# feixue94/pram

Hardware: AMD Instinct MI355X
Metric: query images/sec (640x480, 2048 kpts, 7Scenes nc113) (higher is better)
Workload: dtype f32 results via split-fp16 MFMA (f16 x3 products, f32 accumulate); 1 GPU; 7Scenes full hot path: SFD2 extract+sample -> SegNetViT nc113 (15 layers) -> GML match + 20 Sinkhorn iters, 2048 query kpts vs a 2048-kpt reference set; stages=erm; precision=x3, batches_in_flight_per_gpu=3, hipgraph_replay=False, attention_chunk_keys=4096, frame=640x480, keypoints=2048, parallelism=query-sharded x1, one all-gather of result records, matches_last_step=14291, matches_correct_last_step=14288, gather_order_verified=True

## Files before the change

### pram_amd/csrc/gemm_core_x3w.h

```cpp
#pragma once
#include "common.h"
#include "gemm_core_x3.h"
#include <type_traits>

namespace gemmx3w {

using gemmx3::half4;
using gemmx3::half8;
using gemmx3::split4;
using gemmx3::swz;

constexpr int BK = 32;
#ifndef PRAM_GEMM_SHADOW
#define PRAM_GEMM_SHADOW 1
#endif
constexpr bool SHADOW = PRAM_GEMM_SHADOW != 0;

static __device__ unsigned long long prof[72];

template <int MI, int WM, int WN>
struct Cfg {
    static constexpr int NT = 64 * WM * WN;
    static constexpr int BM = WM * 32 * MI;
    static constexpr int BN = WN * 64;
    static constexpr int PA = BM * 8 / NT;
    static constexpr int QA = BM * 4 / NT;
    static constexpr int QB = BN * 4 / NT;
    static constexpr int RA = NT / 8;
    static constexpr int RQ = NT / 4;
};

template <int MI, int WM, int WN>
struct alignas(16) Smem {
    using C = Cfg<MI, WM, WN>;
    _Float16 ah[2][C::BM * BK];
    _Float16 al[2][C::BM * BK];
    _Float16 bh[2][C::BN * BK];
    _Float16 bl[2][C::BN * BK];
};

template <int ROWS, int NWAVES, class RowPtr>
__device__ __forceinline__ void dma_tile(_Float16* lds_hi, _Float16* lds_lo, RowPtr& rowptr) {
    const int lane = threadIdx.x & 63, wave = threadIdx.x >> 6;
    constexpr int PIECES = ROWS / 16;
#pragma unroll
    for (int i = 0; i < (2 * PIECES + NWAVES - 1) / NWAVES; ++i) {
        const int piece = wave + NWAVES * i;
        if (piece < 2 * PIECES) {
            const int plane = piece / PIECES, pc = piece % PIECES;
            const int row = pc * 16 + (lane >> 2);
            const int slot = (lane & 3) ^ ((row >> 2) & 3);
            const _Float16* src = rowptr(row, plane) + slot * 8;
            _Float16* dst = (plane ? lds_lo : lds_hi) + pc * 16 * BK;
            __builtin_amdgcn_global_load_lds(src, dst, 16, 0, 0);
        }
    }
}

template <int MI, int WM, int WN, bool APLANES, int ABL, int DMA, class Adv, class ALoad, class AOk, class BLoad, class BOk, class APtr, class BPtr, class AXf>
__device__ __forceinline__ void mainloop(Smem<MI, WM, WN>& s, Adv& adv, ALoad& la, AOk& oka, BLoad& lb, BOk& okb, APtr& aptr, BPtr& bptr,
                                         int nk, float a_scale, f32x16 (&acc)[MI][2], float& amax, AXf& axf);

template <int MI, int WM, int WN, bool APLANES, int ABL, int DMA, class Adv, class ALoad, class AOk, class BLoad, class BOk, class APtr, class BPtr>
__device__ __forceinline__ void mainloop(Smem<MI, WM, WN>& s, Adv& adv, ALoad& la, AOk& oka, BLoad& lb, BOk& okb, APtr& aptr, BPtr& bptr,
                                         int nk, float a_scale, f32x16 (&acc)[MI][2], float& amax) {
    gemmx3::NoXform none;
    mainloop<MI, WM, WN, APLANES, ABL, DMA>(s, adv, la, oka, lb, okb, aptr, bptr, nk, a_scale, acc, amax, none);
}

template <int MI, int WM, int WN, bool APLANES, int ABL, int DMA, class Adv, class ALoad, class AOk, class BLoad, class BOk, class APtr, class BPtr, class AXf>
__device__ __forceinline__ void mainloop(Smem<MI, WM, WN>& s, Adv& adv, ALoad& la, AOk& oka, BLoad& lb, BOk& okb, APtr& aptr, BPtr& bptr,
                                         int nk, float a_scale, f32x16 (&acc)[MI][2], float& amax, AXf& axf) {
    static_assert(DMA < 2 || APLANES, "A can only travel by DMA when it is already split");
    using C = Cfg<MI, WM, WN>;
    const int tid = threadIdx.x;
    const int lane = tid & 63, wave = tid >> 6;
    const int wm = wave / WN, wn = wave % WN;
    const int r = lane & 31, h = lane >> 5;
    const int arow = tid >> 3, akq = tid & 7;
    const int qrow = tid >> 2, qsl = tid & 3;

#pragma unroll
    for (int mi = 0; mi < MI; ++mi)
#pragma unroll
        for (int ni = 0; ni < 2; ++ni)
#pragma unroll
            for (int e = 0; e < 16; ++e) acc[mi][ni][e] = 0.f;

    constexpr int NA = APLANES ? C::QA : C::PA;
    struct Regs {
        float4 a[APLANES ? 1 : C::PA];
        uint4 ah[APLANES ? C::QA : 1], al[APLANES ? C::QA : 1];
        uint4 bh[C::QB], bl[C::QB];
        unsigned ok;
        int kt;
    };
    auto issue = [&](int kt, Regs& g) {
        g.ok = 0u;
        g.kt = kt;
        if constexpr (DMA < 2 && !(ABL & 16)) {
#pragma unroll
            for (int p = 0; p < NA; ++p) {
                if constexpr (APLANES) { g.ah[p] = la(p, kt, 0); g.al[p] = la(p, kt, 1); }
                else g.a[p] = la(p, kt);
                g.ok |= (oka(p, kt) ? 1u : 0u) << p;
            }
        }
        if constexpr (DMA < 1) {
#pragma unroll
            for (int p = 0; p < C::QB; ++p) { g.bh[p] = lb(p, kt, 0); g.bl[p] = lb(p, kt, 1); g.ok |= (okb(p, kt) ? 1u : 0u) << (8 + p); }
        }
    };
    auto dma = [&](int buf, int kt) {
        if constexpr (DMA >= 1 && !(ABL & 32)) {
            auto bp = [&](int row, int plane) { return bptr(row, plane, kt); };
            dma_tile<C::BN, C::NT / 64>(s.bh[buf], s.bl[buf], bp);
        }
        if constexpr (DMA >= 2) {
            auto ap = [&](int row, int plane) { return aptr(row, plane, kt); };
            dma_tile<C::BM, C::NT / 64>(s.ah[buf], s.al[buf], ap);
        }
    };
    auto dma_wait = [&]() {
        if constexpr (DMA >= 1) asm volatile("s_waitcnt vmcnt(0)" ::: "memory");
    };
    auto commit = [&](int buf, const Regs& g) {
#pragma unroll
        for (int p = 0; p < ((DMA < 2 && !(ABL & 16)) ? NA : 0); ++p) {
            if constexpr (APLANES) {
                const int row = qrow + C::RQ * p;
                uint4 vh = g.ah[p], vl = g.al[p];
                if (!((g.ok >> p) & 1u)) { vh = make_uint4(0u, 0u, 0u, 0u); vl = vh; }
                const int off = row * BK + swz(qsl, row) * 8;
                *reinterpret_cast<uint4*>(&s.ah[buf][off]) = vh;
                *reinterpret_cast<uint4*>(&s.al[buf][off]) = vl;
            } else {
                const int row = arow + C::RA * p;
                float4 v = g.a[p];
                if (!((g.ok >> p) & 1u)) v = make_float4(0.f, 0.f, 0.f, 0.f);
                else axf(v, p, g.kt);
                half4 hi, lo;
                split4(v, a_scale, hi, lo, amax);
                const int off = row * BK + swz(akq >> 1, row) * 8 + (akq & 1) * 4;
                *reinterpret_cast<half4*>(&s.ah[buf][off]) = hi;
                *reinterpret_cast<half4*>(&s.al[buf][off]) = lo;
            }
        }
#pragma unroll
        for (int p = 0; p < (DMA < 1 ? C::QB : 0); ++p) {
            const int row = qrow + C::RQ * p;
            uint4 vh = g.bh[p], vl = g.bl[p];
            if (!((g.ok >> (8 + p)) & 1u)) { vh = make_uint4(0u, 0u, 0u, 0u); vl = vh; }
            const int off = row * BK + swz(qsl, row) * 8;
            *reinterpret_cast<uint4*>(&s.bh[buf][off]) = vh;
            *reinterpret_cast<uint4*>(&s.bl[buf][off]) = vl;
        }
    };
    auto kstep = [&](int cur, int ks) {
        const int arow0 = (wm * 32 * MI + r) * BK, brow0 = (wn * 64 + r) * BK;
        const int slot = swz(2 * ks + h, r) * 8;
        half8 bh[2], bl[2], ah[2], al[2];
#pragma unroll
        for (int ni = 0; ni < 2; ++ni) {
            bh[ni] = *reinterpret_cast<const half8*>(&s.bh[cur][brow0 + ni * 32 * BK + slot]);
            bl[ni] = *reinterpret_cast<const half8*>(&s.bl[cur][brow0 + ni * 32 * BK + slot]);
        }
        ah[0] = *reinterpret_cast<const half8*>(&s.ah[cur][arow0 + slot]);
        al[0] = *reinterpret_cast<const half8*>(&s.al[cur][arow0 + slot]);
#pragma unroll
        for (int mi = 0; mi < MI; ++mi) {
            if (mi + 1 < MI) {
                ah[(mi + 1) & 1] = *reinterpret_cast<const half8*>(&s.ah[cur][arow0 + (mi + 1) * 32 * BK + slot]);
                al[(mi + 1) & 1] = *reinterpret_cast<const half8*>(&s.al[cur][arow0 + (mi + 1) * 32 * BK + slot]);
            }
            __builtin_amdgcn_sched_barrier(0);
#pragma unroll
            for (int ni = 0; ni < 2; ++ni) acc[mi][ni] = __builtin_amdgcn_mfma_f32_32x32x16_f16(al[mi & 1], bh[ni], acc[mi][ni], 0, 0, 0);
#pragma unroll
            for (int ni = 0; ni < 2; ++ni) acc[mi][ni] = __builtin_amdgcn_mfma_f32_32x32x16_f16(ah[mi & 1], bl[ni], acc[mi][ni], 0, 0, 0);
#pragma unroll
            for (int ni = 0; ni < 2; ++ni) acc[mi][ni] = __builtin_amdgcn_mfma_f32_32x32x16_f16(ah[mi & 1], bh[ni], acc[mi][ni], 0, 0, 0);
        }
    };

    if constexpr (MI <= 2) {
        Regs g0, g1;
        adv(0);
        issue(0, g0);
        dma(0, 0);
        if (nk > 1) { adv(1); issue(1, g1); }
        commit(0, g0);
        dma_wait();
        __syncthreads();
        auto step = [&](int kt, Regs& fresh, Regs& next) {
            if (kt + 1 < nk && !(ABL & 1)) dma((kt + 1) & 1, kt + 1);
            if (kt + 2 < nk && !(ABL & 1)) { adv(kt + 2); issue(kt + 2, fresh); }
            __builtin_amdgcn_sched_barrier(0);
            kstep(kt & 1, 0);
            kstep(kt & 1, (ABL & 2) ? 0 : 1);
            __builtin_amdgcn_sched_barrier(0);
            if (kt + 1 < nk && !(ABL & 1)) commit((kt + 1) & 1, next);
            dma_wait();
            __syncthreads();
        };
        for (int kt = 0; kt < nk; kt += 2) {
            step(kt, g0, g1);
            if (kt + 1 < nk) step(kt + 1, g1, g0);
        }
    } else if constexpr ((ABL == 0 || ABL >= 64) && SHADOW && DMA >= 1) {
        static_assert(MI == 4, "one staging piece per 32-row block of the 256-row tile");
        static_assert(2 * (C::BN / 16) <= (C::NT / 64) * MI && 2 * (C::BM / 16) <= (C::NT / 64) * MI, "MI DMA rounds cover the tile");
        Regs g;
        adv(0);
        issue(0, g);
        dma(0, 0);
        commit(0, g);
        dma_wait();
        __syncthreads();
        auto issue_piece = [&](int kt, int p) {
            if (p == 0) { g.ok = 0u; g.kt = kt; }
            if constexpr (DMA < 2) {
                if (p < NA) {
                    if constexpr (APLANES) { g.ah[p] = la(p, kt, 0); g.al[p] = la(p, kt, 1); }
                    else g.a[p] = la(p, kt);
                    g.ok |= (oka(p, kt) ? 1u : 0u) << p;
                }
            }
        };
        auto dma_piece = [&](int buf, int kt, int i) {
            const int wv = threadIdx.x >> 6, ln = threadIdx.x & 63;
            constexpr int NWV = C::NT / 64;
            {
                constexpr int PIECES = C::BN / 16;
                const int piece = wv + NWV * i;
                if (piece < 2 * PIECES) {
                    const int plane = piece / PIECES, pc = piece % PIECES;
                    const int row = pc * 16 + (ln >> 2);
                    const int slot = (ln & 3) ^ ((row >> 2) & 3);
                    __builtin_amdgcn_global_load_lds(bptr(row, plane, kt) + slot * 8, (plane ? s.bl[buf] : s.bh[buf]) + pc * 16 * BK, 16, 0, 0);
                }
            }
            if constexpr (DMA >= 2) {
                constexpr int PIECES = C::BM / 16;
                const int piece = wv + NWV * i;
                if (piece < 2 * PIECES) {
                    const int plane = piece / PIECES, pc = piece % PIECES;
                    const int row = pc * 16 + (ln >> 2);
                    const int slot = (ln & 3) ^ ((row >> 2) & 3);
                    __builtin_amdgcn_global_load_lds(aptr(row, plane, kt) + slot * 8, (plane ? s.al[buf] : s.ah[buf]) + pc * 16 * BK, 16, 0, 0);
                }
            }
        };
        auto commit_piece = [&](int buf, int p) {
            if (p >= NA) return;
            if constexpr (DMA < 2) {
                if constexpr (APLANES) {
                    const int row = qrow + C::RQ * p;
                    uint4 vh = g.ah[p], vl = g.al[p];
                    if (!((g.ok >> p) & 1u)) { vh = make_uint4(0u, 0u, 0u, 0u); vl = vh; }
                    const int off = row * BK + swz(qsl, row) * 8;
                    *reinterpret_cast<uint4*>(&s.ah[buf][off]) = vh;
                    *reinterpret_cast<uint4*>(&s.al[buf][off]) = vl;
                } else {
                    const int row = arow + C::RA * p;
                    float4 v = g.a[p];
                    if (!((g.ok >> p) & 1u)) v = make_float4(0.f, 0.f, 0.f, 0.f);
                    else axf(v, p, g.kt);
                    half4 hi, lo;
// ... 117 lines not shown
```

### pram_amd/csrc/linear.hip

```cpp
#include "gemm_core.h"
#include "gemm_core_f16.h"
#include "gemm_core_x3.h"
#include "gemm_core_x3w.h"
#include "launch.h"

namespace {

struct LinArgs {
    const float* a0; int lda0; int k0;
    const float* a1; int lda1; int k1;
    const float* w;
    const float* bias;
    const float* residual; int ldr;
    float* out; int ldo;
    int m, n;
    float alpha;
    int flags;
    const float* rcos; const float* rsin; int rot_cols;
    long long sa, sw, so;
    int tiles_m, tiles_n;
    void* out16; int ldo16;
    void* out16_lo; float out16_scale;
    const int* lens; int t_pad;
    void* vt_hi; void* vt_lo; int vt_col0, vt_heads, vt_t, vt_tv;
    unsigned int* status;
    float* row_ssq;
    const float* ln_ssq; int ln_parts; const float* ln_gamma; const float* ln_beta; float ln_eps;
    float act_scale = gemmx3::ACT_SCALE;
};

__device__ __forceinline__ float gelu_erf(float t) {
    const float a = fminf(fabsf(t), 6.0f);
    float q = fmaf(-3.327738795633195e-06f, a, 1.992317265830934e-06f);
    q = fmaf(q, a, 0.0006240683724172413f);
    q = fmaf(q, a, -0.0077792988158762455f);
    q = fmaf(q, a, 0.053078699856996536f);
    q = fmaf(q, a, 0.4589627683162689f);
    q = fmaf(q, a, 1.1511503458023071f);
    q = fmaf(q, a, 0.9999977350234985f);
    const float sgm = __builtin_amdgcn_exp2f(-q);
    return t * (t >= 0.f ? 1.0f - sgm : sgm);
}

template <int PA>
struct LnGeluXf {
    const float* gb; int K; int kq;
    float rstd[PA];
    __device__ __forceinline__ void operator()(float4& v, int p, int kt) const {
#if defined(PRAM_LNA_ABLATE) && (PRAM_LNA_ABLATE == 1 || PRAM_LNA_ABLATE == 4)
        (void)p; (void)kt;
#elif defined(PRAM_LNA_ABLATE) && PRAM_LNA_ABLATE == 2
        const int k = kt * 32 + kq * 4;
        const float4 g = *reinterpret_cast<const float4*>(gb + k);
        const float4 b = *reinterpret_cast<const float4*>(gb + K + k);
        const float rs = rstd[p];
        v.x = v.x * rs * g.x + b.x; v.y = v.y * rs * g.y + b.y; v.z = v.z * rs * g.z + b.z; v.w = v.w * rs * g.w + b.w;
#elif defined(PRAM_LNA_ABLATE) && PRAM_LNA_ABLATE == 3
        const float rs = rstd[p];
        (void)kt;
        v.x = gelu_erf(v.x * rs); v.y = gelu_erf(v.y * rs); v.z = gelu_erf(v.z * rs); v.w = gelu_erf(v.w * rs);
#else
        const int k = kt * 32 + kq * 4;
        const float4 g = *reinterpret_cast<const float4*>(gb + k);
        const float4 b = *reinterpret_cast<const float4*>(gb + K + k);
        const float rs = rstd[p];
        v.x = gelu_erf(v.x * rs * g.x + b.x);
        v.y = gelu_erf(v.y * rs * g.y + b.y);
        v.z = gelu_erf(v.z * rs * g.z + b.z);
        v.w = gelu_erf(v.w * rs * g.w + b.w);
#endif
    }
};

__device__ __forceinline__ float ln_rstd(const LinArgs& p, int row, int K) {
    constexpr int QMAX = 16;
    float s = 0.f;
    for (int q0 = 0; q0 < p.ln_parts; q0 += QMAX) {
        float v[QMAX];
#pragma unroll
        for (int i = 0; i < QMAX; ++i) v[i] = p.ln_ssq[(size_t)min(q0 + i, p.ln_parts - 1) * p.m + row];
#pragma unroll
        for (int i = 0; i < QMAX; ++i)
            if (q0 + i < p.ln_parts) s += v[i];
    }
    return 1.0f / sqrtf(s / (float)K + p.ln_eps);
}

__device__ __forceinline__ bool tile_has_rows(const int* __restrict__ lens, int t_pad, int row0, int bm, int m) {
    if (!lens) return true;
    const int rend = min(row0 + bm, m);
    for (int s = row0 / t_pad; s * t_pad < rend; ++s)
        if (max(row0, s * t_pad) - s * t_pad < lens[s]) return true;
    return false;
}

__device__ __forceinline__ bool row_valid(const int* __restrict__ lens, int t_pad, int row, int m) {
    if (row >= m) return false;
    if (!lens) return true;
    const int sq = row / t_pad;
    return row - sq * t_pad < lens[sq];
}

template <int MI, int WN>
__device__ __forceinline__ void linear_epilogue(const LinArgs& p, f32x16 (&acc)[MI][2], float* out, int row0, int col0,
                                                int BM, int BN, _Float16* stage = nullptr) {
    using gemm::acc_row;
    const int tid = threadIdx.x;
    const int mlast = p.m - 1, nlast = p.n - 1;
    const int lane = tid & 63, wave = __builtin_amdgcn_readfirstlane(tid >> 6);
    const int wm = wave / WN, wn = wave % WN;
    const int r = lane & 31, h = lane >> 5;
    const int cbase = col0 + wn * 64;
    const bool rot = (p.flags & PRAM_LIN_ROTARY) && cbase < p.rot_cols;
    const int c0 = cbase + r, c1 = cbase + 32 + r;
    const bool c0ok = c0 < p.n, c1ok = c1 < p.n;
    const int c0c = min(c0, nlast), c1c = min(c1, nlast);
    const float b0 = p.bias ? p.bias[c0c] : 0.f, b1 = p.bias ? p.bias[c1c] : 0.f;
    const bool ragged = p.lens != nullptr;
    const bool full = (row0 + BM <= p.m) && (col0 + BN <= p.n) && !ragged;
    const unsigned unit_alpha = p.alpha == 1.0f;
    float one = 1.0f;
    asm volatile("" : "+s"(one));
    float emax = 0.f;
    int rlimit = p.m;
    bool straddle = false;
    if (ragged) {
        const int sq = row0 / p.t_pad;
        if ((min(row0 + BM, p.m) - 1) / p.t_pad == sq) rlimit = min(p.m, sq * p.t_pad + p.lens[sq]);
        else straddle = true;
    }
    auto rvalid = [&](int row) -> bool { return straddle ? row_valid(p.lens, p.t_pad, row, p.m) : row < rlimit; };
#pragma clang loop unroll(full)
    for (int mi = 0; mi < MI; ++mi) {
        const int rbase = row0 + wm * 32 * MI;
        float rc_[16], rs_[16], q0[16], q1[16];
        if (rot) {
#pragma unroll
            for (int e = 0; e < 16; ++e) {
                const size_t rr = (size_t)min(rbase + acc_row(mi, e, h), mlast) * 32 + r;
                rc_[e] = p.rcos[rr];
                rs_[e] = p.rsin[rr];
            }
        }
        if (p.residual && full) {
            const char* tile = reinterpret_cast<const char*>(p.residual + (size_t)(rbase + 32 * mi) * p.ldr + cbase);
            const unsigned lane_off = ((unsigned)(4 * h) * (unsigned)p.ldr + r) * 4u, ld4 = (unsigned)p.ldr * 4u;
#pragma unroll
            for (int e = 0; e < 16; ++e) {
                const unsigned o = lane_off + (unsigned)((e & 3) + 8 * (e >> 2)) * ld4;
                q0[e] = *reinterpret_cast<const float*>(tile + o);
                q1[e] = *reinterpret_cast<const float*>(tile + o + 128);
            }
        } else if (p.residual) {
#pragma unroll
// ... 429 lines not shown

template <int MI, int WM, int WN, bool APLANES, int ABL = 0, int DMA = 1, bool LNA = false>
__global__ __launch_bounds__(64 * WM * WN, 2) void linear_x3w_kernel(LinArgs p, PlaneArgs a, const _Float16* __restrict__ wh,
                                                                      const _Float16* __restrict__ wl, float inv) {
    using namespace gemmx3w;
    using C = Cfg<MI, WM, WN>;
    constexpr int BM = C::BM, BN = C::BN;
    static_assert(!(LNA && APLANES), "the LayerNorm + GELU transform applies to an fp32 A operand");
    extern __shared__ __attribute__((aligned(16))) unsigned char smem_raw[];
    Smem<MI, WM, WN>& smem = *reinterpret_cast<Smem<MI, WM, WN>*>(smem_raw);
    float* lngb = reinterpret_cast<float*>(smem_raw + sizeof(Smem<MI, WM, WN>));
    const _Float16* a0h = a.a0h;
    const _Float16* a0l = a.a0l;
    const _Float16* a1h = a.a1h;
    const _Float16* a1l = a.a1l;
    const int alda0 = a.lda0, alda1 = a.lda1;
    if constexpr (APLANES) {
        if (const int z = blockIdx.y) {
            a0h += z * p.sa; a0l += z * p.sa; wh += z * p.sw; wl += z * p.sw; p.out += z * p.so;
        }
    }
    const int nblk = p.tiles_m * p.tiles_n;
    const int id = xcd_remap(blockIdx.x, nblk);
    const int tn = id % p.tiles_n, tm = id / p.tiles_n;
    const int K = p.k0 + p.k1;
    const int tid = threadIdx.x;
    const int arow = tid >> 3, akq = tid & 7, qrow = tid >> 2, qsl = tid & 3;
    const int row0 = tm * BM, col0 = tn * BN;
    if (!tile_has_rows(p.lens, p.t_pad, row0, BM, p.m)) return;
    const int mlast = p.m - 1, nlast = p.n - 1;
    size_t boff[C::QB];
#pragma unroll
    for (int pp = 0; pp < C::QB; ++pp) boff[pp] = (size_t)min(col0 + qrow + C::RQ * pp, nlast) * K + qsl * 8;
    auto lb = [&](int pp, int kt, int plane) -> uint4 { return *reinterpret_cast<const uint4*>((plane ? wl : wh) + boff[pp] + kt * BK); };
    auto okb = [&](int pp, int kt) -> bool { return (col0 + qrow + C::RQ * pp) < p.n; };
    auto adv = [](int) {};
    auto bptr = [&](int row, int plane, int kt) -> const _Float16* {
        return (plane ? wl : wh) + (size_t)min(col0 + row, nlast) * K + kt * BK;
    };
    f32x16 acc[MI][2];
    if constexpr (APLANES) {
        size_t aoff0[C::QA], aoff1[C::QA];
#pragma unroll
        for (int pp = 0; pp < C::QA; ++pp) {
            const size_t rc = (size_t)min(row0 + qrow + C::RQ * pp, mlast);
            aoff0[pp] = rc * alda0 + qsl * 8;
            aoff1[pp] = rc * alda1 + qsl * 8;
        }
        auto la = [&](int pp, int kt, int plane) -> uint4 {
            const int k = kt * BK;
            if (k >= p.k0 && p.k1 > 0)
                return *reinterpret_cast<const uint4*>((plane ? a1l : a1h) + aoff1[pp] + (k - p.k0));
            return *reinterpret_cast<const uint4*>((plane ? a0l : a0h) + aoff0[pp] + k);
        };
        auto oka = [&](int pp, int kt) -> bool { return (row0 + qrow + C::RQ * pp) < p.m; };
        auto aptr = [&](int row, int plane, int kt) -> const _Float16* {
            const size_t rc = (size_t)min(row0 + row, mlast);
            const int k = kt * BK;
            if (k >= p.k0 && p.k1 > 0) return (plane ? a1l : a1h) + rc * alda1 + (k - p.k0);
            return (plane ? a0l : a0h) + rc * alda0 + k;
        };
        float amax = 0.f;
        mainloop<MI, WM, WN, true, ABL, (DMA ? 2 : 0)>(smem, adv, la, oka, lb, okb, aptr, bptr, K / BK, p.act_scale, acc, amax);
    } else {
        const float* arow0[C::PA];
        const float* arow1[C::PA];
        unsigned rowok = 0u;
#pragma unroll
        for (int pp = 0; pp < C::PA; ++pp) {
            const int rc = min(row0 + arow + C::RA * pp, mlast);
            arow0[pp] = p.a0 + (size_t)rc * p.lda0;
            arow1[pp] = p.a1 ? p.a1 + (size_t)rc * p.lda1 - p.k0 : arow0[pp];
            rowok |= (row_valid(p.lens, p.t_pad, row0 + arow + C::RA * pp, p.m) ? 1u : 0u) << pp;
        }
        auto la = [&](int pp, int kt) -> float4 {
            const int kc = kt * BK + akq * 4;
            const bool second = (kt * BK >= p.k0) && p.k1 > 0;
            return *reinterpret_cast<const float4*>((second ? arow1[pp] : arow0[pp]) + kc);
        };
        auto oka = [&](int pp, int kt) -> bool { return ((rowok >> pp) & 1u) != 0u; };
        auto aptr = [](int, int, int) -> const _Float16* { return nullptr; };
        float amax = 0.f;
        if constexpr (LNA) {
#if defined(PRAM_LNA_ABLATE) && PRAM_LNA_ABLATE == 4
            LnGeluXf<C::PA> xf0;
            xf0.gb = lngb; xf0.K = K; xf0.kq = akq;
            for (int pp = 0; pp < C::PA; ++pp) xf0.rstd[pp] = 1.0f;
            mainloop<MI, WM, WN, false, ABL, (DMA ? 1 : 0)>(smem, adv, la, oka, lb, okb, aptr, bptr, K / BK, p.act_scale, acc, amax, xf0);
#else
            {
                float gv[2], bv[2];
#pragma unroll
                for (int j = 0; j < 2; ++j) { const int i = min(tid + C::NT * j, K - 1); gv[j] = p.ln_gamma[i]; bv[j] = p.ln_beta[i]; }
#pragma unroll
                for (int j = 0; j < 2; ++j)
                    if (tid + C::NT * j < K) { lngb[tid + C::NT * j] = gv[j]; lngb[K + tid + C::NT * j] = bv[j]; }
            }
            LnGeluXf<C::PA> xf;
            xf.gb = lngb; xf.K = K; xf.kq = akq;
#pragma unroll
            for (int pp = 0; pp < C::PA; ++pp) {
                const float rs = ln_rstd(p, min(row0 + arow + C::RA * pp, mlast), K);
                xf.rstd[pp] = ((rowok >> pp) & 1u) ? rs : 0.f;
            }
            __syncthreads();
            mainloop<MI, WM, WN, false, ABL, (DMA ? 1 : 0)>(smem, adv, la, oka, lb, okb, aptr, bptr, K / BK, p.act_scale, acc, amax, xf);
#endif
        } else {
            mainloop<MI, WM, WN, false, ABL, (DMA ? 1 : 0)>(smem, adv, la, oka, lb, okb, aptr, bptr, ABL == 128 ? 1 : (ABL == 256 && (blockIdx.x & 1) && blockIdx.x < 256) ? K / BK / 2 : K / BK, p.act_scale, acc, amax);
        }
        x3_range_flag(p.status, amax);
    }
    if constexpr (ABL == 64) {
        float sacc = 0.f;
#pragma unroll
        for (int mi = 0; mi < MI; ++mi)
#pragma unroll
            for (int ni = 0; ni < 2; ++ni)
#pragma unroll
                for (int e = 0; e < 16; ++e) sacc += acc[mi][ni][e];
        if (sacc == 1.2345e-30f) p.out[tid] = sacc;
        return;
    }
    unsigned long long te0 = 0ull;
    if constexpr ((ABL & 4) != 0) te0 = __builtin_readcyclecounter();
#pragma unroll
    for (int mi = 0; mi < MI; ++mi)
#pragma unroll
        for (int ni = 0; ni < 2; ++ni)
#pragma unroll
            for (int e = 0; e < 16; ++e) acc[mi][ni][e] *= inv;
    _Float16* stage = (p.out16_lo && p.n % 8 == 0 && p.ldo16 % 8 == 0) ? reinterpret_cast<_Float16*>(smem_raw) : nullptr;
    linear_epilogue<MI, WN>(p, acc, p.out, ABL == 512 ? 0 : row0, col0, BM, BN, stage);
    if constexpr ((ABL & 4) != 0) {
        asm volatile("s_waitcnt vmcnt(0)" ::: "memory");
        if (tid == 0) atomicAdd(&gemmx3w::prof[6], (unsigned long long)__builtin_readcyclecounter() - te0);
    }
}

template <int NV>
__global__ __launch_bounds__(256) void ln_gelu_kernel(const float* __restrict__ x, int ldx, float* __restrict__ y,
                                                      int ldy, const float* __restrict__ gamma,
                                                      const float* __restrict__ beta, int rows, int cols, float eps,
                                                      const int* __restrict__ lens, int t_pad) {
    const int lane = threadIdx.x & 63;
    const int row = blockIdx.x * 4 + (threadIdx.x >> 6);
    if (row >= rows) return;
    if (lens && (row % t_pad) >= lens[row / t_pad]) return;
    float4 v[NV];
    float sum = 0.f;
#pragma unroll
    for (int i = 0; i < NV; ++i) {
        const int c = (i * 64 + lane) * 4;
        v[i] = (c < cols) ? *reinterpret_cast<const float4*>(x + (size_t)row * ldx + c) : make_float4(0, 0, 0, 0);
        sum += (v[i].x + v[i].y) + (v[i].z + v[i].w);
    }
    const float mean = wave_sum(sum) / (float)cols;
    float sq = 0.f;
#pragma unroll
    for (int i = 0; i < NV; ++i) {
        const int c = (i * 64 + lane) * 4;
        if (c < cols) {
            const float a = v[i].x - mean, b = v[i].y - mean, cc = v[i].z - mean, d = v[i].w - mean;
            sq += (a * a + b * b) + (cc * cc + d * d);
        }
    }
// ... 133 lines not shown
    else if (ab == 16) go(linear_x3w_kernel<MI, WM, WN, APLANES, 16>);
    else if (ab == 32) go(linear_x3w_kernel<MI, WM, WN, APLANES, 32>);
    else if (ab == 64) go(linear_x3w_kernel<MI, WM, WN, APLANES, 64>);
    else if (ab == 128) go(linear_x3w_kernel<MI, WM, WN, APLANES, 128>);
    else if (ab == 512) go(linear_x3w_kernel<MI, WM, WN, APLANES, 512>);
    else if (ab == 256) go(linear_x3w_kernel<MI, WM, WN, APLANES, 256>);
    else go(linear_x3w_kernel<MI, WM, WN, APLANES, 3>);
#else
    hipLaunchKernelGGL((linear_x3w_kernel<MI, WM, WN, APLANES>), grid, blk, shm, st, p, a, wh, wl, inv);
#endif
}

template <bool APLANES>
bool launch_linear_x3_wide(LinArgs& p, PlaneArgs& a, const _Float16* wh, const _Float16* wl, float inv, hipStream_t st, int batch = 1) {
    static const char* force = prof_env("PRAM_X3_TILE");
    if (force && force[0] == 'n') return false;
    if (p.n < 256 || (p.k0 + p.k1) % 32 != 0) return false;
    const long big = (long)cdiv(p.m, 256) * cdiv(p.n, 256) * batch, small = (long)cdiv(p.m, 128) * cdiv(p.n, 256) * batch;
    if (!force && small < 192) return false;
    const bool use256 = force ? (force[1] == '2') : (big >= 224 && 100 * cdiv((int)big, 256) <= 55 * cdiv((int)small, 256));
#ifdef PRAM_PROFILING
    if constexpr (!APLANES) {
        if (force && force[0] == 'f') { launch_linear_x3w_t<2, 1, 8, false>(p, a, wh, wl, inv, st, batch); return true; }
    }
#endif
    if (use256) launch_linear_x3w_t<4, 2, 4, APLANES>(p, a, wh, wl, inv, st, batch);
    else launch_linear_x3w_t<2, 2, 4, APLANES>(p, a, wh, wl, inv, st, batch);
    return true;
}

template <bool APLANES>
void launch_linear_split(LinArgs& p, PlaneArgs& a, const void* w_hi, const void* w_lo, float inv, hipStream_t st, int batch = 1) {
    const _Float16* wh = (const _Float16*)w_hi;
    const _Float16* wl = (const _Float16*)w_lo;
    if (launch_linear_x3_wide<APLANES>(p, a, wh, wl, inv, st, batch)) return;
    int mi, wn;
    gemm::choose_tile(p.m, p.n, &mi, &wn);
    dispatch_tile(mi, wn, [&](auto MI, auto WN) {
        if constexpr (APLANES) {
            PRAM_NOTE_LAUNCH("linear_x3p", MI, WN, -1);
            hipLaunchKernelGGL((linear_x3p_kernel<MI, WN>), dim3(set_tiles<gemmx3::Cfg<MI, WN>>(p, p.n), batch), dim3(gemmx3::NT), 0, st, p, a, wh, wl, inv);
        } else {
            launch_linear_x3_t<MI, WN>(p, wh, wl, inv, st);
        }
    });
}

}

extern "C" int pram_linear_x3p_f32(const void* a0_hi, const void* a0_lo, int lda0, int k0, const void* a1_hi, const void* a1_lo,
                                   int lda1, int k1, const void* w_hi, const void* w_lo, float w_scale, const float* bias,
                                   const float* residual, int ldr, float* out, int ldo, void* out_hi, void* out_lo, int ldo16,
                                   int m, int n, float alpha, int flags, const float* rot_cos, const float* rot_sin, int rot_cols,
                                   void* stream) {
    const char* who = "pram_linear_x3p_f32";
    LinArgs p = lin_a_planes(lda0, k0, lda1, k1);
    lin_out(p, bias, residual, ldr, out, ldo, m, n, alpha);
    with_rotary(p, flags, rot_cos, rot_sin, rot_cols);
    with_planes_out(p, out_hi, out_lo, ldo16);
    if (int e = lin_check(who, X3P_RULES, p, a0_hi && a0_lo && w_hi && w_lo && (out || (out_hi && out_lo)), a1_hi && a1_lo, w_scale)) return e;
    if (m == 0) return PRAM_OK;
    PlaneArgs a{(const _Float16*)a0_hi, (const _Float16*)a0_lo, lda0, (const _Float16*)a1_hi, (const _Float16*)a1_lo, lda1};
    const float inv = 1.0f / (arm_split(p) * w_scale);
    launch_linear_split<true>(p, a, w_hi, w_lo, inv, (hipStream_t)stream);
    return pram_launch_status(who);
}

extern "C" int pram_debug_gemm_phases(unsigned long long* out72, int reset) {
    PRAM_REQUIRE(out72, "pram_debug_gemm_phases: null pointer");
    if (hipMemcpyFromSymbol(out72, HIP_SYMBOL(gemmx3w::prof), 72 * sizeof(unsigned long long)) != hipSuccess) return pram_launch_status("pram_debug_gemm_phases");
    if (reset) {
        unsigned long long z[72] = {0};
        if (hipMemcpyToSymbol(HIP_SYMBOL(gemmx3w::prof), z, sizeof(z)) != hipSuccess) return pram_launch_status("pram_debug_gemm_phases");
    }
    return PRAM_OK;
}

static int x3_ssq_parts(int n) { return cdiv(n, 64); }

static int linear_x3_impl(const char* who, LinArgs& p, bool qkv, const void* w_hi, const void* w_lo, float w_scale, void* stream) {
    if (int e = lin_check(who, X3_RULES, p, p.a0 && w_hi && w_lo && (p.out || (p.out16 && p.out16_lo)), p.a1 != nullptr, w_scale)) return e;
    PRAM_REQUIRE(!(p.row_ssq && (p.out16 || qkv)), "%s: row sums go with an fp32 output", who);
    if (p.ln_ssq)
        PRAM_REQUIRE(p.ln_gamma && p.ln_beta && p.ln_parts > 0 && p.k1 == 0 && p.k0 % 32 == 0 && p.k0 <= 1024,
                     "%s: needs gamma / beta / parts, one input segment, K %% 32 == 0, K <= 1024", who);
    if (qkv) {
        PRAM_REQUIRE(p.vt_hi && p.vt_lo && p.out16 && p.out16_lo, "%s: null pointer", who);
        PRAM_REQUIRE(p.vt_t > 0 && p.vt_t % 64 == 0 && p.m % p.vt_t == 0 && (!p.lens || p.t_pad == p.vt_t),
                     "%s: sequences must be a multiple of 64 tokens long (and t_pad == t_seq)", who);
        PRAM_REQUIRE(p.vt_heads > 0 && p.vt_col0 % 64 == 0 && p.n == p.vt_col0 + p.vt_heads * 64 && p.ldo16 >= p.vt_col0,
                     "%s: the value heads must be the last heads * 64 columns", who);
    }
    if (p.m == 0) return PRAM_OK;
    const float inv = 1.0f / (arm_split(p) * w_scale);
    PlaneArgs none{nullptr, nullptr, 0, nullptr, nullptr, 0};
    launch_linear_split<false>(p, none, w_hi, w_lo, inv, (hipStream_t)stream);
    return pram_launch_status(who);
}

extern "C" int pram_linear_x3_f32(const float* a0, int lda0, int k0, const float* a1, int lda1, int k1, const void* w_hi,
                                  const void* w_lo, float w_scale, const float* bias, const float* residual, int ldr,
                                  float* out, int ldo, void* out_hi, void* out_lo, int ldo16, int m, int n, float alpha,
                                  int flags, const float* rot_cos, const float* rot_sin, int rot_cols, void* stream) {
    LinArgs p = lin_dense(a0, lda0, k0, a1, lda1, k1, bias, residual, ldr, out, ldo, m, n, alpha, flags, rot_cos, rot_sin, rot_cols);
    with_planes_out(p, out_hi, out_lo, ldo16);
    return linear_x3_impl("pram_linear_x3_f32", p, false, w_hi, w_lo, w_scale, stream);
}

extern "C" int pram_linear_x3_ragged_f32(const float* a0, int lda0, int k0, const float* a1, int lda1, int k1, const void* w_hi,
                                         const void* w_lo, float w_scale, const float* bias, const float* residual, int ldr,
                                         float* out, int ldo, void* out_hi, void* out_lo, int ldo16, int m, int n, float alpha,
                                         int flags, const float* rot_cos, const float* rot_sin, int rot_cols, const int* lens,
                                         int t_pad, void* stream) {
    LinArgs p = lin_dense(a0, lda0, k0, a1, lda1, k1, bias, residual, ldr, out, ldo, m, n, alpha, flags, rot_cos, rot_sin, rot_cols);
    with_planes_out(p, out_hi, out_lo, ldo16);
    with_ragged(p, lens, t_pad);
    return linear_x3_impl("pram_linear_x3_ragged_f32", p, false, w_hi, w_lo, w_scale, stream);
}

extern "C" int pram_linear_x3_ssq_parts(int m, int n, int k) { (void)m; (void)k; return x3_ssq_parts(n); }

extern "C" int pram_linear_x3_ssq_f32(const float* a0, int lda0, int k0, const float* a1, int lda1, int k1, const void* w_hi, const void* w_lo,
                                      float w_scale, const float* bias, float* out, int ldo, float* row_ssq, int m, int n,
                                      const int* lens, int t_pad, void* stream) {
    PRAM_REQUIRE(row_ssq && out, "pram_linear_x3_ssq_f32: null pointer");
    LinArgs p = lin_a_f32(a0, lda0, k0, a1, lda1, k1);
    lin_out(p, bias, nullptr, 0, out, ldo, m, n, 1.0f);
    with_ragged(p, lens, t_pad);
    p.row_ssq = row_ssq;
    return linear_x3_impl("pram_linear_x3_ssq_f32", p, false, w_hi, w_lo, w_scale, stream);
}

extern "C" int pram_linear_x3_lngelu_f32(const float* hidden, int ldh, int k, const void* w_hi, const void* w_lo, float w_scale, const float* bias,
                                         const float* residual, int ldr, float* out, int ldo, int m, int n, const float* ln_ssq, int parts,
                                         const float* gamma, const float* beta, float eps, const int* lens, int t_pad, void* stream) {
    PRAM_REQUIRE(ln_ssq && out, "pram_linear_x3_lngelu_f32: null pointer");
    PRAM_REQUIRE(n > 64, "pram_linear_x3_lngelu_f32: n = %d must exceed 64 (narrower outputs: pram_layernorm_gelu_f32 + pram_linear_x3_f32)", n);
    LinArgs p = lin_a_f32(hidden, ldh, k, nullptr, 0, 0);
    lin_out(p, bias, residual, ldr, out, ldo, m, n, 1.0f);
    with_ragged(p, lens, t_pad);
    p.ln_ssq = ln_ssq; p.ln_parts = parts; p.ln_gamma = gamma; p.ln_beta = beta; p.ln_eps = eps;
    return linear_x3_impl("pram_linear_x3_lngelu_f32", p, false, w_hi, w_lo, w_scale, stream);
}

extern "C" int pram_linear_x3_qkv_f32(const float* a0, int lda0, int k0, const void* w_hi, const void* w_lo, float w_scale,
                                      const float* bias, void* out_hi, void* out_lo, int ldo16, void* vt_hi, void* vt_lo, int vt_col0,
                                      int heads, int t_seq, int m, int n, int flags, const float* rot_cos, const float* rot_sin,
                                      int rot_cols, const int* lens, void* stream) {
    LinArgs p = lin_dense(a0, lda0, k0, nullptr, 0, 0, bias, nullptr, 0, nullptr, 0, m, n, 1.0f, flags, rot_cos, rot_sin, rot_cols);
    with_planes_out(p, out_hi, out_lo, ldo16);
    with_ragged(p, lens, lens ? t_seq : 0);
    p.vt_hi = vt_hi; p.vt_lo = vt_lo; p.vt_col0 = vt_col0; p.vt_heads = heads; p.vt_t = p.vt_tv = t_seq;
    return linear_x3_impl("pram_linear_x3_qkv_f32", p, true, w_hi, w_lo, w_scale, stream);
}

static void launch_linear_f16(LinArgs& p, const _Float16* w16, hipStream_t st) {
    int mi, wn;
    gemm::choose_tile(p.m, p.n, &mi, &wn);
    dispatch_tile(mi, wn, [&](auto MI_, auto WN) {
        constexpr int MI = WN == 1 ? 1 : MI_;
        PRAM_NOTE_LAUNCH("linear_f16", MI, WN, -1);
        hipLaunchKernelGGL((linear_f16_kernel<MI, WN>), dim3(set_tiles<gemm16::Cfg<MI, WN>>(p, p.n), 1), dim3(gemm16::NT), 0, st, p, w16);
    });
}

static int linear_f16_f32_impl(const char* who, LinArgs& p, const void* w16, void* stream) {
    if (int e = lin_check(who, F16_RULES, p, p.a0 && w16 && (p.out || p.out16), p.a1 != nullptr, 1.0f)) return e;
    if (p.m == 0) return PRAM_OK;
// ... 120 lines not shown
```

Baseline: 623.8 queries/s.

## Interleave LayerNorm-GELU prologue and B DMA into the x3 MFMA k-loop schedule

Adds a specialised mainloop for GEMMs whose A operand gets a LayerNorm-affine plus GELU transform. The transform is split into coefficient load, affine and activation phases. The activation, split-to-fp16 staging, next-tile A loads and B DMA rounds are spread across the MFMA blocks with sched_group_barrier, so VALU and memory work hides under matrix instructions. The A loads switch to 32-bit unsigned offsets, and the host check now requires lda < 2^21 to keep that addressing valid. The cost is extra code complexity, possible register-pressure changes, and a narrower set of allowed shapes.

```diff
diff --git a/pram_amd/csrc/gemm_core_x3w.h b/pram_amd/csrc/gemm_core_x3w.h
--- a/pram_amd/csrc/gemm_core_x3w.h
+++ b/pram_amd/csrc/gemm_core_x3w.h
@@ -1,7 +1,9 @@
 #pragma once
 #include "common.h"
 #include "gemm_core_x3.h"
+#include <cstddef>
 #include <type_traits>
+#include <utility>
 
 namespace gemmx3w {
 
@@ -67,6 +69,14 @@
     gemmx3::NoXform none;
     mainloop<MI, WM, WN, APLANES, ABL, DMA>(s, adv, la, oka, lb, okb, aptr, bptr, nk, a_scale, acc, amax, none);
 }
+
+template <class AXf, class = void> struct InParts : std::false_type {};
+template <class AXf> struct InParts<AXf, std::void_t<decltype(&AXf::coeffs), decltype(&AXf::affine), decltype(&AXf::act)>> : std::true_type {};
+
+template <class F, int... I>
+__device__ __forceinline__ void static_for_impl(F&& f, std::integer_sequence<int, I...>) { (f(std::integral_constant<int, I>{}), ...); }
+template <int N, class F>
+__device__ __forceinline__ void static_for(F&& f) { static_for_impl(f, std::make_integer_sequence<int, N>{}); }
 
 template <int MI, int WM, int WN, bool APLANES, int ABL, int DMA, class Adv, class ALoad, class AOk, class BLoad, class BOk, class APtr, class BPtr, class AXf>
 __device__ __forceinline__ void mainloop(Smem<MI, WM, WN>& s, Adv& adv, ALoad& la, AOk& oka, BLoad& lb, BOk& okb, APtr& aptr, BPtr& bptr,
@@ -183,7 +193,147 @@
         }
     };
 
-    if constexpr (MI <= 2) {
+    if constexpr (InParts<AXf>::value && !APLANES && DMA == 1 && SHADOW && ABL == 0) {
+        static_assert(C::PA == MI, "one staged quad per 32-row block");
+        static_assert(MI == 4 || MI == 2, "the block schedules below");
+        constexpr int NWV = C::NT / 64, BPIECES = C::BN / 16, BROUNDS = 2 * BPIECES / NWV;
+        static_assert(2 * BPIECES % NWV == 0 && BROUNDS % MI == 0, "whole DMA rounds, spread evenly over the blocks of k-step 0");
+        struct Quads { float4 a[MI]; };
+        Quads g0, g1;
+        unsigned ok = 0u;
+        auto load = [&](int kt, Quads& g) {
+#pragma unroll
+            for (int p = 0; p < MI; ++p) g.a[p] = la(p, kt);
+        };
+        auto stage = [&](int buf, int p, float4 v) {
+            if (!((ok >> p) & 1u)) v = make_float4(0.f, 0.f, 0.f, 0.f);
+            half4 hi, lo;
+            split4(v, a_scale, hi, lo, amax);
+            const int row = arow + C::RA * p;
+            const int off = row * BK + swz(akq >> 1, row) * 8 + (akq & 1) * 4;
+            *reinterpret_cast<half4*>(&s.ah[buf][off]) = hi;
+            *reinterpret_cast<half4*>(&s.al[buf][off]) = lo;
+        };
+        constexpr int RPP = BPIECES / NWV;
+        static_assert(BPIECES % NWV == 0, "a DMA round stays inside one plane");
+        unsigned bdelta[RPP];
+#pragma unroll
+        for (int j = 0; j < RPP; ++j) {
+            const int row = (wave + NWV * j) * 16 + (lane >> 2);
+            const int slot = (lane & 3) ^ ((row >> 2) & 3);
+            bdelta[j] = (unsigned)((bptr(row, 0, 0) + slot * 8) - bptr(0, 0, 0)) * 2u;
+        }
+        auto dma_round = [&](int buf, int kt, int i) {
+            const int plane = i / RPP, pc = wave + NWV * (i % RPP);
+            const char* src = reinterpret_cast<const char*>(bptr(0, plane, kt)) + bdelta[i % RPP];
+            __builtin_amdgcn_global_load_lds(reinterpret_cast<const _Float16*>(src), (plane ? s.bl[buf] : s.bh[buf]) + pc * 16 * BK, 16, 0, 0);
+        };
+        const _Float16* lds = reinterpret_cast<const _Float16*>(&s);
+        constexpr int AL0 = 2 * C::BM * BK, BH0 = 4 * C::BM * BK, BL0 = BH0 + 2 * C::BN * BK;
+        using S = Smem<MI, WM, WN>;
+        static_assert(offsetof(S, al) == AL0 * 2 && offsetof(S, bh) == BH0 * 2 && offsetof(S, bl) == BL0 * 2, "Smem's planes");
+        static_assert((AL0 + 2 * C::BM * BK) * 2 <= 65536 &&(BL0 - BH0 + 2 * C::BN * BK) * 2 <= 65536, "constants within a ds_read's immediate");
+        int afr[2], bfr[2];
+#pragma unroll
+        for (int ks = 0; ks < 2; ++ks) {
+            const int slot = swz(2 * ks + h, r) * 8;
+            afr[ks] = (wm * 32 * MI + r) * BK + slot;
+            bfr[ks] = BH0 + (wn * 64 + r) * BK + slot;
+            asm volatile("" : "+v"(bfr[ks]));
+        }
+        auto loads_landed = [&]() { __builtin_amdgcn_s_waitcnt(0x0F70); };
+#pragma unroll
+        for (int p = 0; p < MI; ++p) ok |= (oka(p, 0) ? 1u : 0u) << p;
+        adv(0);
+        load(0, g0);
+        dma(0, 0);
+        if (nk > 1) { adv(1); load(1, g1); }
+#pragma unroll
+        for (int p = 0; p < MI; ++p) {
+            float4 v = g0.a[p];
+            axf(v, p, 0);
+            stage(0, p, v);
+        }
+        loads_landed();
+        __syncthreads();
+        auto first = [](int b) constexpr -> int {
+            if (MI == 4) return b == 0 ? 0 : (2 * (b - 1) < 12 ? 2 * (b - 1) : 12);
+            return b == 0 ? 0 : b == 1 ? 1 : b == 2 ? 3 : b == 3 ? 5 : 6;
+        };
+        auto step = [&](int kt, Quads& fresh, Quads& next, auto more_t, auto more2_t) {
+            constexpr bool MORE = decltype(more_t)::value, MORE2 = decltype(more2_t)::value;
+            const int cur = kt & 1, nb = cur ^ 1;
+            if constexpr (MORE2) adv(kt + 2);
+            float4 cg = make_float4(0.f, 0.f, 0.f, 0.f), cb = cg;
+            if constexpr (MORE) axf.coeffs(kt + 1, cg, cb);
+            static_for<2>([&](auto ks_t) {
+                constexpr int ks = decltype(ks_t)::value;
+                half8 bh[2], bl[2], ah[2], al[2];
+                auto afrag = [&](int plane, int mi) { return *reinterpret_cast<const half8*>(&lds[afr[ks] + plane * AL0 + cur * (C::BM * BK) + mi * 32 * BK]); };
+                auto bfrag = [&](int plane, int ni) { return *reinterpret_cast<const half8*>(&lds[bfr[ks] + plane * (BL0 - BH0) + cur * (C::BN * BK) + ni * 32 * BK]); };
+#pragma unroll
+                for (int ni = 0; ni < 2; ++ni) { bh[ni] = bfrag(0, ni); bl[ni] = bfrag(1, ni); }
+                ah[0] = afrag(0, 0);
+                al[0] = afrag(1, 0);
+                static_for<MI>([&](auto mi_t) {
+                    constexpr int mi = decltype(mi_t)::value, blk = ks * MI + mi;
+                    if constexpr (mi + 1 < MI) { ah[(mi + 1) & 1] = afrag(0, mi + 1); al[(mi + 1) & 1] = afrag(1, mi + 1); }
+                    __builtin_amdgcn_sched_barrier(0);
+#pragma unroll
+                    for (int ni = 0; ni < 2; ++ni) acc[mi][ni] = __builtin_amdgcn_mfma_f32_32x32x16_f16(al[mi & 1], bh[ni], acc[mi][ni], 0, 0, 0);
+#pragma unroll
+                    for (int ni = 0; ni < 2; ++ni) acc[mi][ni] = __builtin_amdgcn_mfma_f32_32x32x16_f16(ah[mi & 1], bl[ni], acc[mi][ni], 0, 0, 0);
+#pragma unroll
+                    for (int ni = 0; ni < 2; ++ni) acc[mi][ni] = __builtin_amdgcn_mfma_f32_32x32x16_f16(ah[mi & 1], bh[ni], acc[mi][ni], 0, 0, 0);
+                    if constexpr (MORE) {
+                        if constexpr (blk == 0) {
+#pragma unroll
+                            for (int p = 0; p < MI; ++p) axf.affine(next.a[p], p, cg, cb);
+                        }
+                        constexpr int u0 = first(blk), u1 = first(blk + 1);
+                        static_for<u1 - u0>([&](auto j_t) {
+                            constexpr int u = u0 + decltype(j_t)::value, p = u / 3, kind = u % 3;
+                            if constexpr (kind == 0) { next.a[p].x = axf.act(next.a[p].x); next.a[p].y = axf.act(next.a[p].y); }
+                            else if constexpr (kind == 1) { next.a[p].z = axf.act(next.a[p].z); next.a[p].w = axf.act(next.a[p].w); }
+                            else stage(nb, p, next.a[p]);
+                        });
+                        constexpr int LD0 = MI == 4 ? 2 : 0;
+                        constexpr bool ldblk = MORE2 && blk >= LD0 && blk < LD0 + MI;
+                        if constexpr (ks == 0) {
+#pragma unroll
+                            for (int j = 0; j < BROUNDS / MI; ++j) dma_round(nb, kt + 1, mi * (BROUNDS / MI) + j);
+                        }
+                        if constexpr (ldblk) fresh.a[blk - LD0] = la(blk - LD0, kt + 2);
+#pragma unroll
+                        for (int i = 0; i < 6; ++i) {
+                            __builtin_amdgcn_sched_group_barrier(0x008, 1, blk);
+                            __builtin_amdgcn_sched_group_barrier(0x006, 10, blk);
+                            if (ldblk && i == 4) __builtin_amdgcn_sched_group_barrier(0x020, 1, blk);
+                            if (ks == 0 && i == 5) __builtin_amdgcn_sched_group_barrier(0x020, BROUNDS / MI, blk);
+                        }
+                    }
+                });
+            });
+            loads_landed();
+            __syncthreads();
+        };
+        constexpr std::true_type yes{};
+        constexpr std::false_type no{};
+        if (nk > 1) {
+            int kt = 0;
+            for (; kt + 3 < nk; kt += 2) {
+                step(kt, g0, g1, yes, yes);
+                step(kt + 1, g1, g0, yes, yes);
+            }
+            if (kt + 2 < nk) {
+                step(kt, g0, g1, yes, yes);
+                g1 = g0;
+                ++kt;
+            }
+            step(kt, g0, g1, yes, no);
+        }
+        step(nk - 1, g0, g1, no, no);
+    } else if constexpr (MI <= 2) {
         Regs g0, g1;
         adv(0);
         issue(0, g0);
diff --git a/pram_amd/csrc/linear.hip b/pram_amd/csrc/linear.hip
--- a/pram_amd/csrc/linear.hip
+++ b/pram_amd/csrc/linear.hip
@@ -70,6 +70,16 @@
         v.w = gelu_erf(v.w * rs * g.w + b.w);
 #endif
     }
+    __device__ __forceinline__ void coeffs(int kt, float4& g, float4& b) const {
+        const int k = kt * 32 + kq * 4;
+        g = *reinterpret_cast<const float4*>(gb + k);
+        b = *reinterpret_cast<const float4*>(gb + K + k);
+    }
+    __device__ __forceinline__ void affine(float4& v, int p, const float4& g, const float4& b) const {
+        const float rs = rstd[p];
+        v.x = v.x * rs * g.x + b.x; v.y = v.y * rs * g.y + b.y; v.z = v.z * rs * g.z + b.z; v.w = v.w * rs * g.w + b.w;
+    }
+    __device__ __forceinline__ float act(float t) const { return gelu_erf(t); }
 };
 
 __device__ __forceinline__ float ln_rstd(const LinArgs& p, int row, int K) {
@@ -665,6 +675,13 @@
         auto aptr = [](int, int, int) -> const _Float16* { return nullptr; };
         float amax = 0.f;
         if constexpr (LNA) {
+            const char* abase = reinterpret_cast<const char*>(p.a0 + (size_t)row0 * p.lda0);
+            const unsigned astride = (unsigned)p.lda0 * 4u * (unsigned)C::RA;
+            const unsigned aoff0 = (unsigned)arow * (unsigned)p.lda0 * 4u + (unsigned)akq * 16u;
+            const unsigned aofflast = (unsigned)(mlast - row0) * (unsigned)p.lda0 * 4u + (unsigned)akq * 16u;
+            auto la = [&](int pp, int kt) -> float4 {
+                return *reinterpret_cast<const float4*>(abase + (min(aoff0 + (unsigned)pp * astride, aofflast) + (unsigned)(kt * BK * 4)));
+            };
 #if defined(PRAM_LNA_ABLATE) && PRAM_LNA_ABLATE == 4
             LnGeluXf<C::PA> xf0;
             xf0.gb = lngb; xf0.K = K; xf0.kq = akq;
@@ -964,8 +981,8 @@
     if (int e = lin_check(who, X3_RULES, p, p.a0 && w_hi && w_lo && (p.out || (p.out16 && p.out16_lo)), p.a1 != nullptr, w_scale)) return e;
     PRAM_REQUIRE(!(p.row_ssq && (p.out16 || qkv)), "%s: row sums go with an fp32 output", who);
     if (p.ln_ssq)
-        PRAM_REQUIRE(p.ln_gamma && p.ln_beta && p.ln_parts > 0 && p.k1 == 0 && p.k0 % 32 == 0 && p.k0 <= 1024,
-                     "%s: needs gamma / beta / parts, one input segment, K %% 32 == 0, K <= 1024", who);
+        PRAM_REQUIRE(p.ln_gamma && p.ln_beta && p.ln_parts > 0 && p.k1 == 0 && p.k0 % 32 == 0 && p.k0 <= 1024 && p.lda0 < (1 << 21),
+                     "%s: needs gamma / beta / parts, one input segment, K %% 32 == 0, K <= 1024, lda < 2^21", who);
     if (qkv) {
         PRAM_REQUIRE(p.vt_hi && p.vt_lo && p.out16 && p.out16_lo, "%s: null pointer", who);
         PRAM_REQUIRE(p.vt_t > 0 && p.vt_t % 64 == 0 && p.m % p.vt_t == 0 && (!p.lens || p.t_pad == p.vt_t),
```

Result: no change. 628.1 queries/s (median of 6 runs) (+0.7%).
